# kuailehaha/liuzhou

Measured on AMD Instinct MI355X. Metric: self-play positions/sec (fixed sims/move), higher is better.
Workload: dtype f16

## Files before the change

### liuzhou_amd/csrc/lz_engine.hip

```cpp
#include <hip/hip_runtime.h>
#include <hip/amd_detail/amd_hip_unsafe_atomics.h>
#include <math.h>
#include <stdint.h>

#include <mutex>

#include "lz_rng.h"
#include "lz_tree_dev.h"

namespace {

__global__ __launch_bounds__(kBlock) void pack_states_kernel(LzStateSoA s, int64_t B, Packed* __restrict__ out) {
    const int64_t i = (int64_t)blockIdx.x * kBlock + threadIdx.x;
    if (i >= B) return;
    State st;
    st.black = cells_equal(s.board + i * 36, 1);
    st.white = cells_equal(s.board + i * 36, -1);
    st.mb = cells_nonzero(s.marks_black + i * 36);
    st.mw = cells_nonzero(s.marks_white + i * 36);
    st.phase = (int)s.phase[i]; st.player = (int)s.current_player[i];
    st.pm_req = (int)s.pending_marks_required[i]; st.pm_rem = (int)s.pending_marks_remaining[i];
    st.pc_req = (int)s.pending_captures_required[i]; st.pc_rem = (int)s.pending_captures_remaining[i];
    st.forced = (int)s.forced_removals_done[i]; st.move_count = (int)s.move_count[i];
    st.msc = (int)s.moves_since_capture[i];
    out[i] = pack(st);
}

__global__ __launch_bounds__(kBlock) void packed_planes_kernel(const Packed* __restrict__ states, int64_t B,
                                                               float* __restrict__ out) {
    const int lane = lane_id();
    const int64_t g = (int64_t)blockIdx.x * kWavesPerBlock + __builtin_amdgcn_readfirstlane((int)(threadIdx.x >> 6));
    if (g >= B) return;
    const State s = unpack(states[g]);
    const bool blk = s.player == 1;
    const uint64_t own = blk ? s.black : s.white, opp = blk ? s.white : s.black;
    const uint64_t sm = blk ? s.mb : s.mw, om = blk ? s.mw : s.mb;
    float4* orow = reinterpret_cast<float4*>(out + g * 396);
    for (int j = lane; j < 99; j += kWave) {
        const int plane = j / 9, cell0 = (j - plane * 9) * 4;
        uint32_t bits;
        if (plane < 4) {
            const uint64_t src = plane == 0 ? own : plane == 1 ? opp : plane == 2 ? sm : om;
            bits = (uint32_t)(src >> cell0) & 0xFu;
        } else bits = (s.phase == plane - 3) ? 0xFu : 0u;
        orow[j] = make_float4((bits & 1) ? 1.f : 0.f, (bits & 2) ? 1.f : 0.f, (bits & 4) ? 1.f : 0.f, (bits & 8) ? 1.f : 0.f);
    }
}

__global__ __launch_bounds__(kBlock) void tree_begin_kernel(Tree t) {
    const int g = blockIdx.x * kBlock + threadIdx.x;
    if (g >= t.B) return;
    begin_game(t, g);
}


__global__ __launch_bounds__(kBlock) void pos_clear_kernel(int* __restrict__ tab, int64_t n) {
    for (int64_t i = (int64_t)blockIdx.x * kBlock + threadIdx.x; i < n / 4; i += (int64_t)gridDim.x * kBlock)
        reinterpret_cast<int4*>(tab)[i] = make_int4(-1, -1, -1, -1);
}

__global__ __launch_bounds__(kBlock) void tree_select_kernel(Tree t) {
    const int g = wave_game();
    if (g >= t.B) return;
    tree_select(t, g, lane_id(), load_root_info(t, g));
}


template <bool IS_ROOT, bool COMPACT = false>
__global__ __launch_bounds__(kBlock) void tree_expand_kernel(Tree t, const float* __restrict__ lp1,
                                                             const float* __restrict__ lp2,
                                                             const float* __restrict__ lpm,
                                                             const float* __restrict__ priors220,
                                                             const float* __restrict__ values,
                                                             const float* __restrict__ noise, int noise_stride,
                                                             float epsilon, int step) {
    LZ_EXPAND_SCRATCH(sc);
    const int g = wave_game();
    if (g >= t.B) return;
    ptrdiff_t o = 0;
    if (COMPACT) o = (ptrdiff_t)(t.leaf_kind[g] == kLeafExpand ? t.live_row[g] : 0) - g;
    tree_expand<IS_ROOT>(t, g, lane_id(), lp1 ? lp1 + o * 36 : nullptr, lp2 ? lp2 + o * 36 : nullptr,
                         lpm ? lpm + o * 36 : nullptr, priors220 ? priors220 + o * 220 : nullptr, values + o, noise,
                         noise_stride, epsilon, sc, nullptr, step);
}

constexpr int kScanBlock = 1024;
constexpr int kScanUnroll = 8;
__global__ __launch_bounds__(kScanBlock) void tree_live_scan_kernel(Tree t, unsigned long long* __restrict__ count) {
    __shared__ int wave_total[kScanBlock / kWave];
    const int tid = threadIdx.x, lane = tid & (kWave - 1), w = tid / kWave;
    const int rounds = (t.B + kScanBlock - 1) / kScanBlock;
    int cnt = 0;
    for (int r0 = 0; r0 < rounds; r0 += kScanUnroll) {
        int kind[kScanUnroll];
#pragma unroll
        for (int u = 0; u < kScanUnroll; ++u) {
            const int g = (r0 + u) * kScanBlock + tid;
            kind[u] = (r0 + u < rounds && g < t.B) ? t.leaf_kind[g] : kLeafInactive;
        }
#pragma unroll
        for (int u = 0; u < kScanUnroll; ++u) cnt += kind[u] == kLeafExpand ? 1 : 0;
    }
    int incl = cnt;
#pragma unroll
    for (int d = 1; d < kWave; d <<= 1) {
        const int v = __shfl_up(incl, d, kWave);
        if (lane >= d) incl += v;
    }
    if (lane == kWave - 1) wave_total[w] = incl;
    __syncthreads();
    int before = 0, total = 0;
    for (int i = 0; i < kScanBlock / kWave; ++i) { if (i < w) before += wave_total[i]; total += wave_total[i]; }
    int row = before + incl - cnt;
    for (int r0 = 0; r0 < rounds; r0 += kScanUnroll) {
        int kind[kScanUnroll];
        Packed st[kScanUnroll];
#pragma unroll
        for (int u = 0; u < kScanUnroll; ++u) {
            const int g = (r0 + u) * kScanBlock + tid;
            const bool in = r0 + u < rounds && g < t.B;
            kind[u] = in ? t.leaf_kind[g] : kLeafInactive;
            if (in) st[u] = load_state(&t.leaf_state[g]);
        }
#pragma unroll
        for (int u = 0; u < kScanUnroll; ++u) {
            if (kind[u] != kLeafExpand) continue;
            const int g = (r0 + u) * kScanBlock + tid;
            t.live_row[g] = row;
            t.live_state[row] = st[u];
            ++row;
        }
    }
    if (tid == 0) *count = (unsigned long long)total;
}

template <bool IS_ROOT, bool COMPACT = false>
__global__ __launch_bounds__(kBlock) void tree_expand_select_kernel(Tree t, const float* __restrict__ lp1,
                                                                    const float* __restrict__ lp2,
                                                                    const float* __restrict__ lpm,
                                                                    const float* __restrict__ values,
                                                                    const float* __restrict__ noise, int noise_stride,
                                                                    float epsilon, int step) {
#ifndef LZ_EXP_NO_TREE_PRIO
    __builtin_amdgcn_s_setprio(3);
#endif
    LZ_EXPAND_SCRATCH(sc);
    const int g = wave_game();
    if (g >= t.B) return;
    const int lane = lane_id();
    RootInfo root;
    ptrdiff_t o = 0;
    if (COMPACT) o = (ptrdiff_t)(t.leaf_kind[g] == kLeafExpand ? t.live_row[g] : 0) - g;
#ifdef LZ_EXP_TREE_STAMPS
    const unsigned long long lz_t0 = __builtin_readcyclecounter();
#endif
    tree_expand<IS_ROOT>(t, g, lane, lp1 + o * 36, lp2 + o * 36, lpm + o * 36, nullptr, values + o, noise, noise_stride,
                         epsilon, sc, &root, step, nullptr, nullptr LZ_TSTAMP_PASS);
    __threadfence_block();
    if (IS_ROOT) root = load_root_info(t, g);
    LZ_TSTAMP(g, 7)
    tree_select(t, g, lane, root, -1, -1, nullptr LZ_TSTAMP_PASS);
#ifdef LZ_EXP_TREE_STAMPS
    LZ_TADD(g, 19, 1)
#endif
}

constexpr int kSplitMaxGames = 8192;
template <bool COMPACT>
__global__ __launch_bounds__(kBlock) void tree_expand_select_split_kernel(Tree t, const float* __restrict__ lp1,
                                                                          const float* __restrict__ lp2,
                                                                          const float* __restrict__ lpm,
                                                                          const float* __restrict__ values, int step) {
    __builtin_amdgcn_s_setprio(3);
    LZ_EXPAND_SCRATCH(sc);
    __shared__ int s_flag[kWavesPerBlock / 2];
    const int wv = __builtin_amdgcn_readfirstlane((int)(threadIdx.x >> 6));
    const int pair = wv >> 1, role = wv & 1;
    const int g = blockIdx.x * (kWavesPerBlock / 2) + pair;
    const int lane = lane_id();
    if (role == 0 && lane == 0) s_flag[pair] = 0;
    __syncthreads();
    if (g >= t.B) return;
    volatile int* flag = &s_flag[pair];
    ptrdiff_t o = 0;
    if (COMPACT) o = (ptrdiff_t)(t.leaf_kind[g] == kLeafExpand ? t.live_row[g] : 0) - g;
    if (role == 0) {
        tree_expand<false, 1>(t, g, lane, lp1 + o * 36, lp2 + o * 36, lpm + o * 36, nullptr, values + o, nullptr, 0, 0.f, sc,
                              nullptr, step, flag);
        __builtin_amdgcn_fence(__ATOMIC_RELEASE, "workgroup");
        if (lane == 0) *flag = kSplitExpanded;
    } else {
        RootInfo root;
        SplitInfo split;
        tree_expand<false, 2>(t, g, lane, lp1 + o * 36, lp2 + o * 36, lpm + o * 36, nullptr, values + o, nullptr, 0, 0.f, sc,
                              &root, step, flag, &split);
        __threadfence_block();
        split_wait(flag, kSplitInputsRead);
        tree_select(t, g, lane, root, split.wait_edge, split.nolegal_edge, flag);
    }
}

constexpr int kWaveDepth = 160;
struct WaveArrays {
    int K, cap;
    int* path; int* path_len; int* leaf_kind; Packed* leaf_state; float* leaf_value; int* leaf_edge; int* leaf_parent;
    int* sims_done; int* unfinished;
    int* eval_row; Packed* eval_state; unsigned long long* eval_count;
    unsigned long long* eval_total;
    int max_back;
};
struct Level { int e0, ne_pl, parent_n, node; double last_sc; int last_k, in_edge; };
static_assert(sizeof(Level) == 32, "level record is 32 bytes");

__device__ __forceinline__ Tree slot_view(const Tree& t, const WaveArrays& w, int j) {
    Tree v = t;
    const size_t o = (size_t)j * t.B;
    v.path = w.path + o * w.cap; v.path_cap = w.cap; v.path_len = w.path_len + o; v.leaf_kind = w.leaf_kind + o;
    v.leaf_state = w.leaf_state + o; v.leaf_value = w.leaf_value + o; v.leaf_edge = w.leaf_edge + o;
    v.leaf_parent = w.leaf_parent + o;
    return v;
}

__device__ __forceinline__ void tree_select_wave(const Tree& t, const WaveArrays& w, int g, int lane,
                                                 const RootInfo& root, int sims, Level* stack, int* leaf_node,
                                                 int* leaf_act) {
    const int done = w.sims_done[g];
    int to_collect = sims - done;
    to_collect = to_collect < w.K ? to_collect : w.K;
    const bool live = t.root_terminal[g] == 0 && root.ne > 0 && to_collect > 0;
    const Node* nodes = t.nodes + (size_t)g * t.node_cap;
    const Edge* edges = t.edges;
    int found = 0;
    if (live) {
        int d = 0;
        int e0 = root.e0, ne = root.ne, parent_n = root.visits, node_player = root.player, node = 0;
        double last_sc = INFINITY;
        int last_k = -1;
        Edge mine[2];
        double sc[2] = {0.0, 0.0};
        bool loaded = false;
        int ups = 0;
        bool last_leaf = false;
        while (found < to_collect) {
            if (!loaded) {
                const double sq = sqrt((double)(parent_n > 1 ? parent_n : 1));
#pragma unroll
                for (int r = 0; r < 2; ++r) {
                    const int k = r * kWave + lane;
                    sc[r] = __builtin_nan("");
                    if (k < ne) {
                        mine[r] = load_edge(&edges[(size_t)(e0 + k)]);
                        const int n = edge_n(mine[r].n_info);
                        double q = 0.0;
                        if (n > 0) {
                            const double mv = mine[r].W / (double)n;
                            const int child_player = (edge_info(mine[r].n_info) & kInfoWhite) ? -1 : 1;
                            q = child_player == node_player ? mv : -mv;
                        }
                        const double u = t.c_puct * (double)mine[r].P * sq / (1.0 + (double)n);
                        sc[r] = q + u;
                    }
                }
                loaded = true;
            }
            double best = -INFINITY;
            int best_k = -1;
#pragma unroll
            for (int r = 0; r < 2; ++r) {
// ... 857 lines not shown
    if (d->num_games == 0) return LZ_OK;
    const Tree t = no_share(make_tree(d));
    if (is_root)
        hipLaunchKernelGGL(tree_expand_kernel<true>, dim3(gw(t.B)), dim3(kBlock), 0, as_stream(stream), t, lp1, lp2,
                           lpmc, priors220, values, noise, (int)noise_stride, epsilon, -1);
    else
        hipLaunchKernelGGL(tree_expand_kernel<false>, dim3(gw(t.B)), dim3(kBlock), 0, as_stream(stream), t, lp1, lp2,
                           lpmc, priors220, values, nullptr, 0, 0.f, -1);
    return st();
}

int lz_tree_finish(const LzTreeDesc* d, const float* temperatures, const float* target_temperatures,
                   float prior_pseudocount, const uint8_t* force_uniform, int sample_moves, const float* uniforms,
                   float* policy_dense,
                   int32_t* chosen_index, int32_t* chosen_code, uint8_t* chosen_valid, uint8_t* terminal_mask,
                   float* root_value, int32_t* child_count, int32_t* child_action, int32_t* child_visits,
                   float* child_prior, int64_t out_cap, void* stream) {
    if (!tree_ok(d) || !temperatures || !policy_dense || !chosen_index || !chosen_code || !chosen_valid ||
        !terminal_mask || !root_value || !child_count || !child_action || !child_visits || !child_prior || out_cap < 1)
        return LZ_ERR_ARG;
    if (d->num_games == 0) return LZ_OK;
    if (!(prior_pseudocount >= 0.f) || ((force_uniform || sample_moves) && !uniforms)) return LZ_ERR_ARG;
    hipLaunchKernelGGL(tree_finish_kernel, dim3(gw(d->num_games)), dim3(kBlock), 0, as_stream(stream), make_tree(d),
                       temperatures, target_temperatures, prior_pseudocount, force_uniform, sample_moves, uniforms, policy_dense, chosen_index, reinterpret_cast<int4*>(chosen_code),
                       chosen_valid, terminal_mask, root_value, child_count, child_action, child_visits, child_prior,
                       (int)out_cap);
    return st();
}

static long long* g_advance_ticks = nullptr;
int lz_debug_advance_ticks(int64_t* ticks) { g_advance_ticks = reinterpret_cast<long long*>(ticks); return LZ_OK; }

int lz_prof_aux_begin(int kind, void* stream);
int lz_prof_aux_end(int kind, void* stream, int64_t units);

int lz_tree_advance(const LzTreeDesc* d, const int32_t* played_action, const uint8_t* reset, int64_t next_sims,
                    int32_t* dropped, int32_t* pruned, void* stream) {
    if (!tree_ok(d) || next_sims < 0) return LZ_ERR_ARG;
    if (d->num_games == 0) return LZ_OK;
    const int words = (d->node_cap + kWave - 1) / kWave;
    if (words > kMarkWordsBig) return LZ_ERR_UNSUPPORTED;
    const int64_t rn = next_sims + 1;
    if (rn > d->node_cap) return LZ_ERR_ARG;
    if ((int64_t)d->chunk_cap * (d->edge_chunk - (kMaxChildren - 1)) < (int64_t)d->node_cap * kMaxChildren) return LZ_ERR_ARG;
    const bool big = words > kMarkWordsMax;
    const int wpb = big ? 1 : kWavesPerBlock;
    const size_t lds = (size_t)wpb * (words * (sizeof(uint64_t) + sizeof(int)) + 3 * kWave * sizeof(int));
    if (big) {
        static std::mutex mu;
        static bool configured[64] = {};
        int dev = 0;
        if (hipGetDevice(&dev) != hipSuccess || dev < 0 || dev >= 64) return LZ_ERR_LAUNCH;
        std::lock_guard<std::mutex> lk(mu);
        if (!configured[dev]) {
            const size_t most = (size_t)kMarkWordsBig * (sizeof(uint64_t) + sizeof(int)) + 3 * kWave * sizeof(int);
            if (hipFuncSetAttribute(reinterpret_cast<const void*>(tree_advance_kernel<1>),
                                    hipFuncAttributeMaxDynamicSharedMemorySize, (int)most) != hipSuccess) {
                (void)hipGetLastError();
                return LZ_ERR_LAUNCH;
            }
            configured[dev] = true;
        }
    }
    (void)lz_prof_aux_begin(1, stream);
    if (big)
        hipLaunchKernelGGL(tree_advance_kernel<1>, dim3((unsigned)d->num_games), dim3(kWave), lds, as_stream(stream), make_tree(d),
                           played_action, reset, (int)rn, words, dropped, pruned, g_advance_ticks);
    else
        hipLaunchKernelGGL(tree_advance_kernel<kWavesPerBlock>, dim3(gw(d->num_games)), dim3(kBlock), lds, as_stream(stream),
                           make_tree(d), played_action, reset, (int)rn, words, dropped, pruned, g_advance_ticks);
    (void)lz_prof_aux_end(1, stream, d->num_games);
    return st();
}

static int tree_search_impl(const LzTreeDesc* d, const LzNetDesc* net, int64_t sims, float* planes, float* lp1,
                            float* lp2, float* lpmc, float* values, const float* noise, int64_t noise_stride,
                            float epsilon, bool continue_trees, void* stream) {
    if (!tree_ok(d) || !net || sims < 0 || !lp1 || !lp2 || !lpmc || !values) return LZ_ERR_ARG;
    const int64_t B = d->num_games;
    if (B == 0) return LZ_OK;
    int rc = continue_trees ? LZ_OK : lz_tree_begin(d, stream);
    if (rc) return rc;
    (void)planes;
    const Tree t = split_step(B) ? no_share(make_tree(d)) : make_tree(d);
    if (t.live_count != nullptr) {
        if (d->live_count_cap < sims + 2) return LZ_ERR_ARG;
        hipLaunchKernelGGL(tree_live_scan_kernel, dim3(1), dim3(kScanBlock), 0, as_stream(stream), t, t.live_count);
        for (int64_t s = 0; s <= sims; ++s) {
            rc = lz_net_forward_packed_counted_f16(net, d->live_state, B, d->live_count + s, lp1, lp2, lpmc, nullptr, values,
                                                   stream);
            if (rc) return rc;
            if (s == sims) {
                if (s == 0)
                    hipLaunchKernelGGL((tree_expand_kernel<true, true>), dim3(gw(t.B)), dim3(kBlock), 0, as_stream(stream), t,
                                       lp1, lp2, lpmc, (const float*)nullptr, values, noise, (int)noise_stride, epsilon, (int)s);
                else
                    hipLaunchKernelGGL((tree_expand_kernel<false, true>), dim3(gw(t.B)), dim3(kBlock), 0, as_stream(stream), t,
                                       lp1, lp2, lpmc, (const float*)nullptr, values, (const float*)nullptr, 0, 0.f, (int)s);
            } else if (s == 0) {
                hipLaunchKernelGGL((tree_expand_select_kernel<true, true>), dim3(gw(t.B)), dim3(kBlock), 0, as_stream(stream),
                                   t, lp1, lp2, lpmc, values, noise, (int)noise_stride, epsilon, (int)s);
            } else {
                (void)lz_prof_aux_begin(0, stream);
                if (split_step(t.B))
                    hipLaunchKernelGGL((tree_expand_select_split_kernel<true>), dim3(gw2(t.B)), dim3(kBlock), 0,
                                       as_stream(stream), t, lp1, lp2, lpmc, values, (int)s);
                else
                    hipLaunchKernelGGL((tree_expand_select_kernel<false, true>), dim3(gw(t.B)), dim3(kBlock), 0, as_stream(stream),
                                       t, lp1, lp2, lpmc, values, nullptr, 0, 0.f, (int)s);
                (void)lz_prof_aux_end(0, stream, B);
            }
            if (s < sims)
                hipLaunchKernelGGL(tree_live_scan_kernel, dim3(1), dim3(kScanBlock), 0, as_stream(stream), t,
                                   t.live_count + (s + 1));
        }
        return st();
    }
    for (int64_t s = 0; s <= sims; ++s) {
        rc = lz_net_forward_packed_f16(net, d->leaf_state, B, lp1, lp2, lpmc, nullptr, values, stream);
        if (rc) return rc;
        if (s == sims) {
            if (s == 0)
                hipLaunchKernelGGL(tree_expand_kernel<true>, dim3(gw(t.B)), dim3(kBlock), 0, as_stream(stream), t, lp1, lp2,
                                   lpmc, (const float*)nullptr, values, noise, (int)noise_stride, epsilon, (int)s);
            else
                hipLaunchKernelGGL(tree_expand_kernel<false>, dim3(gw(t.B)), dim3(kBlock), 0, as_stream(stream), t, lp1, lp2,
                                   lpmc, (const float*)nullptr, values, (const float*)nullptr, 0, 0.f, (int)s);
        } else if (s == 0) {
            hipLaunchKernelGGL(tree_expand_select_kernel<true>, dim3(gw(t.B)), dim3(kBlock), 0, as_stream(stream), t, lp1,
                               lp2, lpmc, values, noise, (int)noise_stride, epsilon, (int)s);
        } else {
            (void)lz_prof_aux_begin(0, stream);
            if (split_step(t.B))
                hipLaunchKernelGGL((tree_expand_select_split_kernel<false>), dim3(gw2(t.B)), dim3(kBlock), 0, as_stream(stream),
                                   t, lp1, lp2, lpmc, values, (int)s);
            else
                hipLaunchKernelGGL(tree_expand_select_kernel<false>, dim3(gw(t.B)), dim3(kBlock), 0, as_stream(stream), t, lp1,
                                   lp2, lpmc, values, nullptr, 0, 0.f, (int)s);
            (void)lz_prof_aux_end(0, stream, B);
        }
    }
    return st();
}

#ifdef LZ_EXP_TREE_STAMPS
LZ_API int lz_exp_tree_stamps(unsigned long long* out32, int reset) {
    if (out32 && hipMemcpyFromSymbol(out32, HIP_SYMBOL(g_tree_stamps), 32 * sizeof(unsigned long long)) != hipSuccess) return LZ_ERR_LAUNCH;
    if (reset) {
        unsigned long long z[32] = {};
        if (hipMemcpyToSymbol(HIP_SYMBOL(g_tree_stamps), z, sizeof(z)) != hipSuccess) return LZ_ERR_LAUNCH;
    }
    return LZ_OK;
}
#endif

int64_t lz_tree_desc_bytes(void) { return (int64_t)sizeof(LzTreeDesc); }

int lz_root_prepare(const void* root_states, int64_t B, const float* lp1, const float* lp2, const float* lpmc,
                    const float* noise, float epsilon, int64_t* legal_index_mat, float* priors_mat,
                    int32_t* action_code_mat, uint8_t* valid_mask, int32_t* counts, uint8_t* terminal_mask,
                    float* leaf_mat, void* child_states, int32_t* child_ref, uint64_t* n_children,
                    int64_t child_capacity, int32_t* overflow, void* stream) {
    if (B < 0) return LZ_ERR_ARG;
    if (B == 0) return LZ_OK;
    if (!root_states || !lp1 || !lp2 || !lpmc || !legal_index_mat || !priors_mat || !action_code_mat || !valid_mask ||
        !counts || !terminal_mask || !leaf_mat || !child_states || !child_ref || !n_children || child_capacity < 0)
        return LZ_ERR_ARG;
    if (reinterpret_cast<uintptr_t>(action_code_mat) & 15) return LZ_ERR_ALIGN;
    hipLaunchKernelGGL(zero_u64_kernel, dim3(1), dim3(64), 0, as_stream(stream),
                       reinterpret_cast<unsigned long long*>(n_children));
    hipLaunchKernelGGL(root_prepare_kernel, dim3(gw(B)), dim3(kBlock), 0, as_stream(stream),
                       reinterpret_cast<const Packed*>(root_states), B, lp1, lp2, lpmc, noise, epsilon, legal_index_mat,
                       priors_mat, reinterpret_cast<int4*>(action_code_mat), valid_mask, counts, terminal_mask, leaf_mat,
                       reinterpret_cast<Packed*>(child_states), child_ref,
                       reinterpret_cast<unsigned long long*>(n_children), child_capacity, overflow);
    return st();
}

int lz_root_collect(const void* root_states, const void* child_states, const int32_t* child_ref,
                    const float* child_values, const uint64_t* n_children, int64_t capacity, float soft_value_k,
                    float* leaf_mat, void* stream) {
    if (capacity < 0) return LZ_ERR_ARG;
    if (capacity == 0) return LZ_OK;
    if (!root_states || !child_states || !child_ref || !child_values || !n_children || !leaf_mat) return LZ_ERR_ARG;
    hipLaunchKernelGGL(root_collect_kernel, dim3(1024), dim3(kBlock), 0, as_stream(stream),
                       reinterpret_cast<const Packed*>(root_states), reinterpret_cast<const Packed*>(child_states),
                       child_ref, child_values, reinterpret_cast<const unsigned long long*>(n_children), capacity,
                       soft_value_k, leaf_mat);
    return st();
}

int lz_root_topk_children(const void* root_states, int64_t B, const float* leaf_mat, const uint8_t* valid_mask,
                          const int32_t* action_code_mat, int64_t top_k, int32_t* top_slot, void* l2_states, void* stream) {
    if (B < 0 || top_k < 0 || top_k > kRootCap) return LZ_ERR_ARG;
    if (B == 0 || top_k == 0) return LZ_OK;
    if (!root_states || !leaf_mat || !valid_mask || !action_code_mat || !top_slot || !l2_states) return LZ_ERR_ARG;
    if (reinterpret_cast<uintptr_t>(action_code_mat) & 15) return LZ_ERR_ALIGN;
// ... 97 lines not shown
```

### liuzhou_amd/csrc/lz_tree_dev.h

```cpp
#pragma once
#include <hip/hip_runtime.h>
#include <hip/amd_detail/amd_hip_unsafe_atomics.h>
#include <math.h>
#include <stdint.h>

#include "lz_soa.h"
#include "lz_wave.h"

using namespace lz;

namespace {

constexpr int kWave = 64;
constexpr int kBlock = 256;
constexpr int kWavesPerBlock = 4;
constexpr int kMaxChildren = 72;

enum LeafKind : int { kLeafInactive = 0, kLeafExpand = 1, kLeafTerminal = 2, kLeafReusedRoot = 3, kLeafShared = 4 };
constexpr uint8_t kInfoWhite = 1;
constexpr uint8_t kInfoTerminal = 2;

struct Edge {
    double W;
    float P;
    uint32_t n_info;
    int32_t child;
    int32_t cbegin;
    uint8_t act;
    uint8_t cn;
    uint8_t pad[6];
};
static_assert(sizeof(Edge) == 32, "edge record is 32 bytes");
struct Node {
    Packed state;
    int32_t edge_begin, nedges;
    int32_t parent;
    int32_t old_begin;
};
static_assert(sizeof(Node) == 48, "node record is 48 bytes");
__device__ __forceinline__ int edge_n(uint32_t ni) { return (int)(ni & 0xFFFFFFu); }
__device__ __forceinline__ uint8_t edge_info(uint32_t ni) { return (uint8_t)(ni >> 24); }

struct Tree {
    int B, node_cap, chunk, path_cap, chunk_cap;
    const Packed* root_state;
    Node* nodes; Edge* edges;
    int* n_nodes; int* n_edges;
    int* chunk_list; int* n_chunks; int* free_chunks; int* pool_top;
    int* pool_stats;
    int* root_visits; double* root_W; float* root_init_value;
    int* path; int* path_len; int* leaf_kind; Packed* leaf_state; float* leaf_value;
    uint8_t* root_terminal; const uint8_t* active;
    int* leaf_edge; int* leaf_parent;
    double c_puct;
    int fast_select;
    int* trace_kind; Packed* trace_leaf; float* trace_heads; float* trace_priors; float* trace_value;
    int trace_cap;
    int* eval_count;
    Packed* live_state; int* live_row; unsigned long long* live_count;
    int* pos_index; float* node_value; int* leaf_src; int* share_count;
    int pos_slots, share;
};

typedef unsigned int u32x4 __attribute__((ext_vector_type(4)));
__device__ __forceinline__ Edge load_edge(const Edge* p) {
    const u32x4* q = reinterpret_cast<const u32x4*>(p);
    union U { u32x4 v[2]; Edge e; __device__ U() {} } u;
    u.v[0] = q[0]; u.v[1] = q[1];
    return u.e;
}
__device__ __forceinline__ Packed load_state(const Packed* p) {
    const u32x4* q = reinterpret_cast<const u32x4*>(p);
    union U { u32x4 v[2]; Packed s; __device__ U() {} } u;
    u.v[0] = q[0]; u.v[1] = q[1];
    return u.s;
}
constexpr uint32_t kPathFlip = 0x80000000u;

__device__ __forceinline__ int lane_id() { return threadIdx.x & 63; }
__device__ __forceinline__ int wave_game() {
    return blockIdx.x * kWavesPerBlock + __builtin_amdgcn_readfirstlane((int)(threadIdx.x >> 6));
}
__device__ __forceinline__ bool same_state(const Packed& a, const Packed& b) {
    return a.w0 == b.w0 && a.w1 == b.w1 && a.w2 == b.w2 && a.w3 == b.w3;
}
__device__ __forceinline__ uint32_t pos_hash(const Packed& s) {
    uint64_t h = s.w0 * 0x9E3779B97F4A7C15ull;
    h = (h ^ (h >> 29) ^ s.w1) * 0xBF58476D1CE4E5B9ull;
    h = (h ^ (h >> 31) ^ s.w2) * 0x94D049BB133111EBull;
    h = (h ^ (h >> 27) ^ s.w3) * 0x9E3779B97F4A7C15ull;
    return (uint32_t)(h >> 32);
}
struct PosWindow { int entry; int first_empty; uint32_t base; };
__device__ __forceinline__ PosWindow pos_window(const Tree& t, int g, const Packed& s, int nn, int lane) {
    const int* tab = t.pos_index + (size_t)g * t.pos_slots;
    const uint32_t mask = (uint32_t)t.pos_slots - 1u;
    PosWindow w;
    w.base = pos_hash(s) & mask;
    w.entry = tab[(w.base + (uint32_t)lane) & mask];
    const uint64_t em = __ballot(w.entry < 1 || w.entry >= nn);
    w.first_empty = em ? __ffsll((unsigned long long)em) - 1 : kWave;
    return w;
}
__device__ __forceinline__ int pos_find(const Tree& t, int g, const Packed& s, int nn, int lane) {
    const PosWindow w = pos_window(t, g, s, nn, lane);
    bool hit = false;
    if (lane < w.first_empty) hit = same_state(load_state(&t.nodes[(size_t)g * t.node_cap + w.entry].state), s);
    const uint64_t hm = __ballot(hit);
    return hm ? lzw::lane_bcast(w.entry, __ffsll((unsigned long long)hm) - 1) : -1;
}

#ifdef LZ_EXP_TREE_STAMPS
__device__ unsigned long long g_tree_stamps[32];
#define LZ_TSTAMP_ON(g) ((g) == 5)
#define LZ_TSTAMP(g, k) if (LZ_TSTAMP_ON(g)) { asm volatile("s_waitcnt vmcnt(0) lgkmcnt(0)" ::: "memory"); \
        if (lane_id() == 0) { atomicAdd(&g_tree_stamps[k], (unsigned long long)__builtin_readcyclecounter() - lz_t0); \
                              atomicAdd(&g_tree_stamps[20 + (k)], 1ull); } }
#define LZ_TSTAMP_ARG , unsigned long long lz_t0 = 0
#define LZ_TSTAMP_PASS , lz_t0
#define LZ_TCLOCK(g, var) unsigned long long var = 0; if (LZ_TSTAMP_ON(g)) { asm volatile("s_waitcnt vmcnt(0) lgkmcnt(0)" ::: "memory"); var = __builtin_readcyclecounter(); }
#define LZ_TADD(g, k, v) if (LZ_TSTAMP_ON(g) && lane_id() == 0) atomicAdd(&g_tree_stamps[k], (unsigned long long)(v));
#else
#define LZ_TSTAMP(g, k)
#define LZ_TCLOCK(g, var)
#define LZ_TADD(g, k, v)
#define LZ_TSTAMP_ARG
#define LZ_TSTAMP_PASS
#endif

__device__ __forceinline__ double terminal_value_for_mover(const State& s) {
    const int st = game_status(s);
    if (st == 1 || st == -1) return st == s.player ? 1.0 : -1.0;
    return 0.0;
}


__device__ __forceinline__ void release_chunks(const Tree& t, int g, int keep) {
    const int nc = t.n_chunks[g];
    if (nc > keep) {
        const int base = atomicAdd(t.pool_top, nc - keep);
        const int* list = t.chunk_list + (size_t)g * t.chunk_cap;
        for (int i = keep; i < nc; ++i) t.free_chunks[base + (i - keep)] = list[i];
    }
    t.n_chunks[g] = keep < nc ? keep : nc;
}
__device__ __forceinline__ void release_chunks_wave(const Tree& t, int g, int keep, int lane) {
    const int nc = t.n_chunks[g];
    if (nc > keep) {
        int base = 0;
        if (lane == 0) base = atomicAdd(t.pool_top, nc - keep);
        base = __builtin_amdgcn_readfirstlane(base);
        const int* list = t.chunk_list + (size_t)g * t.chunk_cap;
        for (int i = keep + lane; i < nc; i += kWave) t.free_chunks[base + (i - keep)] = list[i];
        if (lane == 0) t.n_chunks[g] = keep;
    }
}
__device__ __forceinline__ bool root_pending(const Tree& t, int g) {
    return t.n_nodes[g] == 1 && t.nodes[(size_t)g * t.node_cap].nedges < 0 && t.root_terminal[g] == 0;
}

__device__ __forceinline__ int take_chunk(const Tree& t, int g, bool for_root = false) {
    const int nc = t.n_chunks[g];
    if (nc >= t.chunk_cap) { atomicAdd(t.pool_stats, 1); return -1; }
    const int top = atomicSub(t.pool_top, 1) - 1;
    const int reserved = for_root ? 0 : __atomic_load_n(t.pool_stats + 2, __ATOMIC_RELAXED);
    if (top < reserved) { atomicAdd(t.pool_top, 1); atomicAdd(t.pool_stats, 1); return -1; }
    if (for_root && root_pending(t, g)) atomicSub(t.pool_stats + 2, 1);
    atomicMin(t.pool_stats + 1, top);
    const int cid = t.free_chunks[top];
    t.chunk_list[(size_t)g * t.chunk_cap + nc] = cid;
    t.n_chunks[g] = nc + 1;
    return cid * t.chunk;
}

__device__ __forceinline__ void begin_game(const Tree& t, int g, bool release = true) {
    const bool was_pending = root_pending(t, g);
    if (release) release_chunks(t, g, 0);
    const Packed rs = t.root_state[g];
    Node& root = t.nodes[(size_t)g * t.node_cap];
    root.state = rs;
    root.edge_begin = 0;
    root.nedges = -1;
    root.parent = -1;
    t.n_nodes[g] = 1;
    t.n_edges[g] = 0;
    t.root_visits[g] = 0;
    t.root_W[g] = 0.0;
    t.root_init_value[g] = 0.f;
// ... 74 lines not shown
                    }
                    const float s = q + cf * mine[r].P * sqf / (1.0f + (float)n);
                    fs[r] = s == s ? s : -INFINITY;
                }
            }
            const float b = fs[1] > fs[0] ? fs[1] : fs[0];
            const float m1 = lzw::wave_max_nonan(b);
            const uint64_t w0 = __ballot(fs[0] == m1), w1 = __ballot(fs[1] == m1);
            if (m1 > -INFINITY && m1 < INFINITY && __popcll(w0) + __popcll(w1) == 1 && __ballot(off_scale) == 0ull) {
                const int c = w0 ? __ffsll((unsigned long long)w0) - 1 : kWave + __ffsll((unsigned long long)w1) - 1;
                const float b2 = (c & 63) == lane ? (c < kWave ? fs[1] : fs[0]) : b;
                const float m2 = lzw::wave_max_nonan(b2);
                if (m1 - m2 > 1e-4f * (1.0f + fabsf(m1))) chosen = c;
            }
        }
        if (chosen < 0) {
            const double sq = sqrt((double)(parent_n > 1 ? parent_n : 1));
            double best = -INFINITY;
            int best_k = -1;
#pragma unroll
            for (int r = 0; r < 2; ++r) {
                if (r == 1 && ne <= kWave) break;
                const int k = r * kWave + lane;
                if (k < ne) {
                    const int n = edge_n(mine[r].n_info);
                    double q = 0.0;
                    if (n > 0) {
                        const double mv = mine[r].W / (double)n;
                        const int child_player = (edge_info(mine[r].n_info) & kInfoWhite) ? -1 : 1;
                        q = child_player == node_player ? mv : -mv;
                    }
                    const double u = t.c_puct * (double)mine[r].P * sq / (1.0 + (double)n);
                    const double sc = q + u;
                    if (sc > best) { best = sc; best_k = k; }
                }
            }
            const double mx = lzw::wave_max(best);
            const uint64_t lo = __ballot(best_k >= 0 && best_k < kWave && best == mx);
            if (lo) chosen = __ffsll((unsigned long long)lo) - 1;
            else {
                const uint64_t hi = __ballot(best_k >= kWave && best == mx);
                if (!hi) break;
                chosen = kWave + __ffsll((unsigned long long)hi) - 1;
            }
        }
        chosen = __builtin_amdgcn_readfirstlane(chosen);
        const int src = chosen & 63;
        const bool up = chosen >= kWave;
        const uint32_t c_ni = (uint32_t)lzw::lane_bcast((int)(up ? mine[1].n_info : mine[0].n_info), src);
        int c_child = lzw::lane_bcast(up ? mine[1].child : mine[0].child, src);
        int c_begin = lzw::lane_bcast(up ? mine[1].cbegin : mine[0].cbegin, src);
        int c_meta = lzw::lane_bcast((int)(up ? mine[1].act : mine[0].act) | ((int)(up ? mine[1].cn : mine[0].cn) << 8), src);
        uint8_t info = edge_info(c_ni);
        if (e0 + chosen == wait_edge) {
            split_wait(flag, kSplitExpanded);
            const Edge fresh = load_edge(&run[chosen]);
            c_child = fresh.child; c_begin = fresh.cbegin;
            c_meta = (int)fresh.act | ((int)fresh.cn << 8);
        }
        if (e0 + chosen == nolegal_edge) info |= kInfoTerminal;
        const int child_player = (info & kInfoWhite) ? -1 : 1;
#ifdef LZ_EXP_TREE_STAMPS
        { LZ_TCLOCK(g, lv_t2) LZ_TADD(g, 17, lv_t2 - lv_t0) LZ_TADD(g, 18, 1) }
#endif
        leaf_edge = e0 + chosen;
        if (lane == 0) path[depth] = leaf_edge | (child_player != node_player ? (int)kPathFlip : 0);
        ++depth;
        if (info & kInfoTerminal) {
            kind = kLeafTerminal;
            term_value = (float)((int)((info >> 2) & 3) - 1);
            break;
        }
        if (c_child < 0) { kind = kLeafExpand; leaf_action = c_meta & 0xFF; break; }
        node_state = load_state(&nodes[c_child].state);
        parent_n = edge_n(c_ni);
        node_player = child_player;
        node = c_child;
        e0 = c_begin;
        ne = c_meta >> 8;
        if (depth >= t.path_cap - 1) break;
    }
    LZ_TSTAMP(g, 8)
    Packed leaf_packed{};
    int src = -1;
    if (kind == kLeafExpand) {
        State leaf = unpack(node_state);
        int kd, p, q2, ex;
        index_to_code(leaf.phase, leaf_action, kd, p, q2, ex);
        apply_legal(leaf, kd, p, q2);
        leaf_packed = pack(leaf);
        if (t.share) {
            src = pos_find(t, g, leaf_packed, t.n_nodes[g], lane);
            if (src > 0) kind = kLeafShared;
        }
    }
    if (lane == 0) {
        t.path_len[g] = depth;
        t.leaf_kind[g] = kind;
        t.leaf_value[g] = term_value;
        t.leaf_edge[g] = leaf_edge;
        t.leaf_parent[g] = node;
        if (kind == kLeafExpand || kind == kLeafShared) t.leaf_state[g] = leaf_packed;
        if (kind == kLeafShared) t.leaf_src[g] = src;
    }
    LZ_TSTAMP(g, 9)
}

struct ExpandScratch { float* val; int* act; };
constexpr int kExpandScratchBytes = 80 * 8;
#define LZ_EXPAND_SCRATCH(name)                                                            \
    __shared__ float name##_val[kWavesPerBlock][80];                                      \
    __shared__ int name##_act[kWavesPerBlock][80];                                        \
    const int name##_wv = __builtin_amdgcn_readfirstlane((int)(threadIdx.x >> 6));        \
    const ExpandScratch name = {name##_val[name##_wv], name##_act[name##_wv]}

struct SplitInfo { int wait_edge, nolegal_edge; };
template <bool IS_ROOT, int ROLE = 0>
__device__ __forceinline__ void tree_expand(const Tree& t, int g, int lane, const float* __restrict__ lp1,
                                            const float* __restrict__ lp2, const float* __restrict__ lpm,
                                            const float* __restrict__ priors220, const float* __restrict__ values,
                                            const float* __restrict__ noise, int noise_stride, float epsilon,
                                            ExpandScratch sc, RootInfo* root_after = nullptr, int step = -1,
                                            volatile int* flag = nullptr, SplitInfo* split = nullptr LZ_TSTAMP_ARG) {
    static_assert(ROLE == 0 || !IS_ROOT, "the root step is never split");
    LZ_TSTAMP(g, 0)
    const int kind = t.leaf_kind[g];
    Node* nodes = t.nodes + (size_t)g * t.node_cap;
    Edge* edges = t.edges;
    const int* path = t.path + (size_t)g * t.path_cap;
    RootInfo root{};
    int plen_ld = 0, leaf_edge = -1, leaf_parent = 0, nn_ld = 0, ne_ld = 0, path_entry = 0;
    double root_w = 0.0;
    float leaf_value_ld = 0.f, value_ld = 0.f;
    Packed leaf_packed = t.leaf_state[g];
    if (!IS_ROOT) {
        root = load_root_info(t, g);
        plen_ld = t.path_len[g];
        leaf_edge = t.leaf_edge[g];
        leaf_parent = t.leaf_parent[g];
        path_entry = lane < t.path_cap ? path[lane] : 0;
        root_w = t.root_W[g];
        leaf_value_ld = t.leaf_value[g];
    }
    nn_ld = t.n_nodes[g];
    ne_ld = t.n_edges[g];
    const bool shared = !IS_ROOT && ROLE == 0 && kind == kLeafShared;
    value_ld = shared ? 0.f : values[g];
    const bool indexed = !IS_ROOT && ROLE != 2 && t.pos_index != nullptr;
    PosWindow pw{0, kWave, 0u};
    if (indexed) pw = pos_window(t, g, leaf_packed, nn_ld, lane);
    int src_begin = 0;
    if (shared) {
        const int src = t.leaf_src[g];
        value_ld = t.node_value[(size_t)g * t.node_cap + src];
        src_begin = nodes[src].edge_begin;
    }
    if (root_after != nullptr) *root_after = root;
    if (ROLE == 1) {
        asm volatile("s_waitcnt vmcnt(0)" ::: "memory");
        if (lane == 0) *flag = kSplitInputsRead;
    }
    if (ROLE == 2) { split->wait_edge = -1; split->nolegal_edge = -1; }
    LZ_TSTAMP(g, 1)
    const bool tracing = ROLE != 2 && t.trace_kind != nullptr && step >= 0 && step < t.trace_cap;
    const size_t tslot = tracing ? (size_t)step * (size_t)t.B + (size_t)g : 0;
    if (tracing) {
        if (lane == 0) { t.trace_kind[tslot] = kind; t.trace_leaf[tslot] = leaf_packed; t.trace_value[tslot] = value_ld; }
        for (int a = lane; a < 220; a += kWave) t.trace_priors[tslot * 220 + a] = 0.f;
    }
    if (kind == kLeafInactive) return;
    if (kind == kLeafReusedRoot) {
        if (IS_ROOT && noise != nullptr) {
            const int ne = nodes[0].nedges, e0 = nodes[0].edge_begin;
            if (ne > 1) {
                const float keep = (float)(1.0 - (double)epsilon);
                float pr[2]; bool ok[2];
#pragma unroll
                for (int r = 0; r < 2; ++r) {
                    const int k = r * kWave + lane;
                    ok[r] = k < ne;
                    pr[r] = ok[r] ? keep * edges[(size_t)(e0 + k)].P + epsilon * noise[(size_t)g * noise_stride + k] : 0.f;
                }
                float psum = 0.f;
#pragma unroll
                for (int r = 0; r < 2; ++r) {
                    uint64_t m = __ballot(ok[r]);
                    while (m) {
                        const int l = __builtin_amdgcn_readfirstlane(__ffsll((unsigned long long)m) - 1);
                        psum += lzw::lane_bcast(pr[r], l);
                        m &= m - 1;
                    }
                }
                const float denom = psum < 1e-8f ? 1e-8f : psum;
#pragma unroll
                for (int r = 0; r < 2; ++r)
                    if (ok[r]) edges[(size_t)(e0 + r * kWave + lane)].P = pr[r] / denom;
            }
        }
        return;
    }
    const int plen = IS_ROOT ? 0 : plen_ld;
    double backup_value = 0.0;

    if (kind == kLeafTerminal) {
        backup_value = (double)leaf_value_ld;
    } else {
        if (shared) { if (t.share_count != nullptr && lane == 0) t.share_count[g] += 1; }
        else if (ROLE != 2 && t.eval_count != nullptr && lane == 0) t.eval_count[g] += 1;
        const State s = unpack(leaf_packed);
        const Legal L = legal_actions(s, 0);
        const int n = legal_count(L);
        if (ROLE == 2) {
            backup_value = n == 0 ? -1.0 : (double)value_ld;
            if (n == 0) split->nolegal_edge = leaf_edge; else split->wait_edge = leaf_edge;
        } else if (n == 0) {
            backup_value = -1.0;
            if (lane == 0) {
                if (IS_ROOT) {
                    if (root_pending(t, g)) atomicSub(t.pool_stats + 2, 1);
                    nodes[0].nedges = 0; t.root_terminal[g] = 1; t.root_init_value[g] = -1.f;
                }
                else atomicOr(&edges[(size_t)leaf_edge].n_info, (uint32_t)kInfoTerminal << 24);
            }
        } else {
            float h1 = 0.f, h2 = 0.f, hm = 0.f;
            const bool heads = priors220 == nullptr;
            if (heads && lane < kCells && !shared) {
                h1 = lp1[(size_t)g * 36 + lane]; h2 = lp2[(size_t)g * 36 + lane]; hm = lpm[(size_t)g * 36 + lane];
                if (tracing) {
                    float* th = t.trace_heads + tslot * 108;
                    th[lane] = h1; th[36 + lane] = h2; th[72 + lane] = hm;
                }
            }
            float val[4]; int slot[4]; bool lg[4];
            int base = 0;
            float mx = -INFINITY;
// ... 3 lines not shown
                lg[it] = a < 217 && legal_bit(L, a);
                val[it] = 0.f; slot[it] = 0;
                const uint64_t bal = __ballot(lg[it]);
                if (bal == 0) continue;
                slot[it] = base + __popcll(bal & ((1ull << lane) - 1ull));
                base += __popcll(bal);
                int from = 0, dest = 0, cell = 0;
                if (a >= 36 && a < 180) { from = (a - 36) >> 2; dest = move_dest(from, (a - 36) & 3); dest = dest < 0 ? 0 : (dest > 35 ? 35 : dest); }
                else if (a >= 180 && a < 216) cell = a - 180;
                else if (a < 36) cell = a;
                float x;
                if (heads) {
                    const float p1d = __shfl(h1, dest), p2f = __shfl(h2, from), p1c = __shfl(h1, cell), pmc = __shfl(hm, cell);
                    x = a < 36 ? p1c : a < 180 ? (p2f + p1d) : a < 216 ? pmc : 0.f;
                } else {
                    x = lg[it] ? priors220[(size_t)g * 220 + a] : 0.f;
                }
                val[it] = x;
                if (heads && lg[it]) mx = fmaxf(mx, x);
            }
            if (heads) {
                mx = lzw::wave_max(mx);
                float sum = 0.f;
#pragma unroll
                for (int it = 0; it < 4; ++it) { val[it] = lg[it] ? expf(val[it] - mx) : 0.f; sum += val[it]; }
                sum = lzw::wave_sum(sum);
#pragma unroll
                for (int it = 0; it < 4; ++it) val[it] = val[it] / sum;
            }
            if (tracing) {
#pragma unroll
                for (int it = 0; it < 4; ++it)
                    if (lg[it]) t.trace_priors[tslot * 220 + it * kWave + lane] = val[it];
            }
            if (IS_ROOT && noise != nullptr && n > 1) {
                const float keep = (float)(1.0 - (double)epsilon);
#pragma unroll
                for (int it = 0; it < 4; ++it)
                    if (lg[it]) val[it] = keep * val[it] + epsilon * noise[(size_t)g * noise_stride + slot[it]];
            }
            LZ_TSTAMP(g, 2)
#pragma unroll
            for (int it = 0; it < 4; ++it)
                if (lg[it]) { sc.val[slot[it]] = val[it]; sc.act[slot[it]] = it * kWave + lane; }
            __builtin_amdgcn_fence(__ATOMIC_RELEASE, "wavefront");
            __builtin_amdgcn_wave_barrier();
            __builtin_amdgcn_fence(__ATOMIC_ACQUIRE, "wavefront");
            float cval[2]; int cact[2];
#pragma unroll
            for (int r = 0; r < 2; ++r) {
                const int k = r * kWave + lane;
                cval[r] = k < n ? sc.val[k] : 0.f;
                cact[r] = k < n ? sc.act[k] : 0;
            }
            float psum = 0.f;
            if (shared) {
#pragma unroll
                for (int r = 0; r < 2; ++r) {
                    const int k = r * kWave + lane;
                    cval[r] = k < n ? edges[(size_t)(src_begin + k)].P : 0.f;
                }
                psum = 1.f;
            } else {
#pragma unroll 4
                for (int k = 0; k < n; ++k) psum += lzw::lane_bcast(k < kWave ? cval[0] : cval[1], k & 63);
            }
            const bool bad = !(psum > 0.f) || !isfinite(psum);
            LZ_TSTAMP(g, 3)
            int node_id = 0, e0 = 0;
            if (lane == 0) {
                e0 = ne_ld;
                const int off = e0 & (t.chunk - 1);
                if (off == 0 || off + n > t.chunk) e0 = take_chunk(t, g, IS_ROOT);
                if (e0 >= 0) {
                    t.n_edges[g] = e0 + n;
                    if (IS_ROOT) node_id = 0;
                    else {
                        node_id = nn_ld; t.n_nodes[g] = node_id + 1;
                        Edge& in = edges[(size_t)leaf_edge];
                        in.child = node_id; in.cbegin = e0; in.cn = (uint8_t)n;
                        nodes[node_id].state = leaf_packed;
                        nodes[node_id].parent = leaf_parent;
                        if (t.node_value != nullptr) t.node_value[(size_t)g * t.node_cap + node_id] = value_ld;
                        if (indexed && !shared && pw.first_empty < kWave)
                            t.pos_index[(size_t)g * t.pos_slots + ((pw.base + (uint32_t)pw.first_empty) & ((uint32_t)t.pos_slots - 1u))] = node_id;
                    }
                    nodes[node_id].edge_begin = e0;
                    nodes[node_id].nedges = n;
                }
                if (IS_ROOT) t.root_init_value[g] = value_ld;
            }
            e0 = __builtin_amdgcn_readfirstlane(e0);
            node_id = __builtin_amdgcn_readfirstlane(node_id);
            const int n_write = e0 >= 0 ? n : 0;
            LZ_TSTAMP(g, 4)
            Edge* new_run = edges + (size_t)(e0 >= 0 ? e0 : 0);
            for (int r = 0; r < (n_write > kWave ? 2 : 1); ++r) {
                const int k = r * kWave + lane;
                if (k >= n_write) continue;
                const int a = r == 0 ? cact[0] : cact[1];
                State c = s;
                int kd, p, q2, ex;
                index_to_code(s.phase, a, kd, p, q2, ex);
                apply_legal(c, kd, p, q2);
                uint8_t info = c.player < 0 ? kInfoWhite : 0;
                if (game_status(c) != 0) {
                    const int tv = (int)terminal_value_for_mover(c);
                    info |= kInfoTerminal | (uint8_t)((tv + 1) << 2);
                }
                Edge rec;
                rec.W = 0.0;
                rec.P = shared ? (r == 0 ? cval[0] : cval[1]) : bad ? (1.0f / (float)n) : ((r == 0 ? cval[0] : cval[1]) / psum);
                rec.n_info = (uint32_t)info << 24;
                rec.child = -1;
                rec.cbegin = 0;
                rec.act = (uint8_t)a;
                rec.cn = 0;
                rec.pad[0] = rec.pad[1] = rec.pad[2] = rec.pad[3] = rec.pad[4] = rec.pad[5] = 0;
                new_run[k] = rec;
            }
            backup_value = (double)value_ld;
            LZ_TSTAMP(g, 5)
        }
    }
    if (IS_ROOT || ROLE == 1) return;
    if (plen > 0) {
        int flips_above = 0;
        for (int hi = plen; hi > 0; hi -= kWave) {
            const int lo = hi > kWave ? hi - kWave : 0;
            const int j = lo + lane;
            const bool in = j < hi;
            const uint32_t pe = !in ? 0u : (lo == 0 ? (uint32_t)path_entry : (uint32_t)path[j]);
            const uint64_t F = __ballot(in && (pe & kPathFlip) != 0u);
            const int above = in ? __popcll(F >> (lane + 1)) : 0;
            if (in) {
                Edge* e = &edges[(size_t)(pe & ~kPathFlip)];
                const double v = ((above + flips_above) & 1) ? -backup_value : backup_value;
                atomicAdd(&e->n_info, 1u);
                unsafeAtomicAdd(&e->W, v);
            }
            flips_above += __popcll(F);
        }
        root.visits += 1;
        if (lane == 0) {
            t.root_visits[g] = root.visits;
            t.root_W[g] = root_w + ((flips_above & 1) ? -backup_value : backup_value);
        }
        if (root_after != nullptr) root_after->visits = root.visits;
    }
    LZ_TSTAMP(g, 6)
}

inline hipStream_t as_stream(void* s) { return reinterpret_cast<hipStream_t>(s); }
inline int st() { return hipGetLastError() == hipSuccess ? LZ_OK : LZ_ERR_LAUNCH; }

Tree make_tree(const LzTreeDesc* d) {
    Tree t;
    t.B = (int)d->num_games; t.node_cap = d->node_cap; t.chunk = d->edge_chunk; t.path_cap = d->path_cap;
    t.chunk_cap = d->chunk_cap;
    t.chunk_list = d->chunk_list; t.n_chunks = d->n_chunks; t.free_chunks = d->free_chunks; t.pool_top = d->pool_top;
    t.pool_stats = d->pool_stats;
    t.root_state = reinterpret_cast<const Packed*>(d->root_state);
    t.nodes = reinterpret_cast<Node*>(d->nodes);
    t.edges = reinterpret_cast<Edge*>(d->edges);
    t.n_nodes = d->n_nodes; t.n_edges = d->n_edges; t.root_visits = d->root_visits; t.root_W = d->root_w;
    t.root_init_value = d->root_init_value;
    t.path = d->path; t.path_len = d->path_len; t.leaf_kind = d->leaf_kind;
    t.leaf_state = reinterpret_cast<Packed*>(d->leaf_state); t.leaf_value = d->leaf_value;
    t.root_terminal = d->root_terminal; t.active = d->active;
    t.leaf_edge = d->leaf_edge; t.leaf_parent = d->leaf_parent;
    t.c_puct = d->exploration_weight;
    { const char* e = getenv("LZ_TREE_F32SEL"); t.fast_select = (e && e[0] == '1'); }
    const bool tr = d->trace_cap > 0 && d->trace_kind && d->trace_leaf && d->trace_heads && d->trace_priors && d->trace_value;
    t.trace_kind = tr ? d->trace_kind : nullptr;
    t.trace_leaf = tr ? reinterpret_cast<Packed*>(d->trace_leaf) : nullptr;
    t.trace_heads = tr ? d->trace_heads : nullptr;
    t.trace_priors = tr ? d->trace_priors : nullptr;
    t.trace_value = tr ? d->trace_value : nullptr;
    t.trace_cap = tr ? (int)d->trace_cap : 0;
    t.eval_count = d->eval_count;
    const bool live = d->live_state && d->live_row && d->live_count && d->live_count_cap > 0;
    t.live_state = live ? reinterpret_cast<Packed*>(d->live_state) : nullptr;
    t.live_row = live ? d->live_row : nullptr;
    t.live_count = live ? reinterpret_cast<unsigned long long*>(d->live_count) : nullptr;
    const bool pos = d->pos_index && d->node_value && d->leaf_src && d->pos_slots >= kWave &&
                     (d->pos_slots & (d->pos_slots - 1)) == 0;
    t.pos_index = pos ? d->pos_index : nullptr;
    t.node_value = pos ? d->node_value : nullptr;
    t.leaf_src = pos ? d->leaf_src : nullptr;
    t.pos_slots = pos ? (int)d->pos_slots : 0;
    t.share_count = d->share_count;
    { const char* e = getenv("LZ_TREE_SHARE"); t.share = pos && !tr && !(e && e[0] == '0') ? 1 : 0; }
    return t;
}
inline Tree no_share(Tree t) { t.share = 0; return t; }
bool tree_ok(const LzTreeDesc* d) {
    return d && d->num_games >= 0 && d->node_cap >= 2 && d->path_cap >= 3 &&
           d->edge_chunk >= 128 && (d->edge_chunk & (d->edge_chunk - 1)) == 0 && d->chunk_cap >= 1 &&
           d->pool_chunks >= 1 && (d->pool_chunks + 1) * (int64_t)d->edge_chunk <= (int64_t)1 << 31 &&
           d->pool_chunks >= d->num_games &&
           d->chunk_list && d->n_chunks && d->free_chunks && d->pool_top && d->pool_stats &&
           d->root_state && d->nodes && d->edges && d->n_nodes && d->n_edges &&
           d->root_visits && d->root_w && d->root_init_value && d->path && d->path_len && d->leaf_kind &&
           d->leaf_state && d->leaf_value && d->root_terminal && d->leaf_edge && d->leaf_parent;
}

}
```

Measured before the change: 11400.

## Parallelize live-leaf compaction across blocks and reuse select-time position-index slot

```diff
diff --git a/liuzhou_amd/csrc/lz_engine.hip b/liuzhou_amd/csrc/lz_engine.hip
--- a/liuzhou_amd/csrc/lz_engine.hip
+++ b/liuzhou_amd/csrc/lz_engine.hip
@@ -78,7 +78,7 @@
     const int g = wave_game();
     if (g >= t.B) return;
     ptrdiff_t o = 0;
-    if (COMPACT) o = (ptrdiff_t)(t.leaf_kind[g] == kLeafExpand ? t.live_row[g] : 0) - g;
+    if (COMPACT) o = (ptrdiff_t)t.live_row[g] - g;
     tree_expand<IS_ROOT>(t, g, lane_id(), lp1 ? lp1 + o * 36 : nullptr, lp2 ? lp2 + o * 36 : nullptr,
                          lpm ? lpm + o * 36 : nullptr, priors220 ? priors220 + o * 220 : nullptr, values + o, noise,
                          noise_stride, epsilon, sc, nullptr, step);
@@ -124,14 +124,81 @@
         }
 #pragma unroll
         for (int u = 0; u < kScanUnroll; ++u) {
+            const int g = (r0 + u) * kScanBlock + tid;
+            if (r0 + u < rounds && g < t.B) t.live_row[g] = kind[u] == kLeafExpand ? row : 0;
             if (kind[u] != kLeafExpand) continue;
-            const int g = (r0 + u) * kScanBlock + tid;
-            t.live_row[g] = row;
             t.live_state[row] = st[u];
             ++row;
         }
     }
     if (tid == 0) *count = (unsigned long long)total;
+}
+
+constexpr int kListBlock = 1024;
+constexpr int kListWaves = kListBlock / kWave;
+constexpr int kListMaxRounds = 256;
+inline bool list_build_ok(const Tree& t) {
+    return (t.B + kScanBlock - 1) / kScanBlock <= kListMaxRounds && (reinterpret_cast<uintptr_t>(t.leaf_kind) & 15) == 0;
+}
+inline unsigned list_groups(int B) { return (unsigned)(((B < kScanBlock ? B : kScanBlock) + kWave - 1) / kWave); }
+__global__ __launch_bounds__(kListBlock) void tree_live_list_kernel(Tree t, unsigned long long* __restrict__ count) {
+    __shared__ uint64_t col_mask[kListMaxRounds];
+    __shared__ int wave_before[kListWaves];
+    const int tid = threadIdx.x, lane = tid & (kWave - 1);
+    const int wv = __builtin_amdgcn_readfirstlane(tid >> 6);
+    const int rounds = (t.B + kScanBlock - 1) / kScanBlock;
+    const int c0 = blockIdx.x * kWave;
+    const int q = c0 >> 2, groups = rounds * q;
+    int before = 0;
+    for (int i0 = tid; i0 < groups; i0 += 4 * kListBlock) {
+        int4 k[4];
+#pragma unroll
+        for (int u = 0; u < 4; ++u) {
+            const int i = i0 + u * kListBlock;
+            const int r = i / (q > 0 ? q : 1);
+            const int g = r * kScanBlock + 4 * (i - r * q);
+            k[u] = make_int4(kLeafInactive, kLeafInactive, kLeafInactive, kLeafInactive);
+            if (i < groups) {
+                if (g + 3 < t.B) k[u] = *reinterpret_cast<const int4*>(t.leaf_kind + g);
+                else {
+                    if (g < t.B) k[u].x = t.leaf_kind[g];
+                    if (g + 1 < t.B) k[u].y = t.leaf_kind[g + 1];
+                    if (g + 2 < t.B) k[u].z = t.leaf_kind[g + 2];
+                }
+            }
+        }
+#pragma unroll
+        for (int u = 0; u < 4; ++u)
+            before += (k[u].x == kLeafExpand) + (k[u].y == kLeafExpand) + (k[u].z == kLeafExpand) + (k[u].w == kLeafExpand);
+    }
+    const int g_first = wv * kScanBlock + c0 + lane;
+    Packed st_first{};
+    if (wv < rounds && g_first < t.B) st_first = load_state(&t.leaf_state[g_first]);
+    for (int r = wv; r < rounds; r += kListWaves) {
+        const int g = r * kScanBlock + c0 + lane;
+        const uint64_t m = __ballot(g < t.B && t.leaf_kind[g] == kLeafExpand);
+        if (lane == 0) col_mask[r] = m;
+    }
+    before = lzw::wave_incl_scan(before);
+    if (lane == kWave - 1) wave_before[wv] = before;
+    __syncthreads();
+    int base = 0;
+    for (int i = 0; i < kListWaves; ++i) base += wave_before[i];
+    const uint64_t below = (1ull << lane) - 1ull;
+    int col_row = base;
+    for (int r = 0; r < rounds; ++r) col_row += __popcll(col_mask[r] & below);
+    for (int r = 0; r < rounds; ++r) {
+        const bool live = (col_mask[r] >> lane) & 1ull;
+        if (r % kListWaves == wv) {
+            const int g = r * kScanBlock + c0 + lane;
+            if (g < t.B) {
+                t.live_row[g] = live ? col_row : 0;
+                if (live) t.live_state[col_row] = r == wv ? st_first : load_state(&t.leaf_state[g]);
+            }
+        }
+        col_row += live ? 1 : 0;
+    }
+    if (blockIdx.x == gridDim.x - 1 && wv == 0 && lane == kWave - 1) *count = (unsigned long long)col_row;
 }
 
 template <bool IS_ROOT, bool COMPACT = false>
@@ -150,7 +217,7 @@
     const int lane = lane_id();
     RootInfo root;
     ptrdiff_t o = 0;
-    if (COMPACT) o = (ptrdiff_t)(t.leaf_kind[g] == kLeafExpand ? t.live_row[g] : 0) - g;
+    if (COMPACT) o = (ptrdiff_t)t.live_row[g] - g;
 #ifdef LZ_EXP_TREE_STAMPS
     const unsigned long long lz_t0 = __builtin_readcyclecounter();
 #endif
@@ -183,7 +250,7 @@
     if (g >= t.B) return;
     volatile int* flag = &s_flag[pair];
     ptrdiff_t o = 0;
-    if (COMPACT) o = (ptrdiff_t)(t.leaf_kind[g] == kLeafExpand ? t.live_row[g] : 0) - g;
+    if (COMPACT) o = (ptrdiff_t)t.live_row[g] - g;
     if (role == 0) {
         tree_expand<false, 1>(t, g, lane, lp1 + o * 36, lp2 + o * 36, lpm + o * 36, nullptr, values + o, nullptr, 0, 0.f, sc,
                               nullptr, step, flag);
@@ -1207,10 +1274,21 @@
     int rc = continue_trees ? LZ_OK : lz_tree_begin(d, stream);
     if (rc) return rc;
     (void)planes;
-    const Tree t = split_step(B) ? no_share(make_tree(d)) : make_tree(d);
+    const char* ref_env = getenv("LZ_TREE_LIST_REF");
+    const bool ref = ref_env && ref_env[0] == '1';
+    Tree t = split_step(B) ? no_share(make_tree(d)) : make_tree(d);
+    t.sel_slot = t.share && !ref ? 1 : 0;
     if (t.live_count != nullptr) {
         if (d->live_count_cap < sims + 2) return LZ_ERR_ARG;
-        hipLaunchKernelGGL(tree_live_scan_kernel, dim3(1), dim3(kScanBlock), 0, as_stream(stream), t, t.live_count);
+        const bool list = !ref && list_build_ok(t);
+        auto build_list = [&](unsigned long long* count) {
+            if (list)
+                hipLaunchKernelGGL(tree_live_list_kernel, dim3(list_groups(t.B)), dim3(kListBlock), 0, as_stream(stream), t,
+                                   count);
+            else
+                hipLaunchKernelGGL(tree_live_scan_kernel, dim3(1), dim3(kScanBlock), 0, as_stream(stream), t, count);
+        };
+        build_list(t.live_count);
         for (int64_t s = 0; s <= sims; ++s) {
             rc = lz_net_forward_packed_counted_f16(net, d->live_state, B, d->live_count + s, lp1, lp2, lpmc, nullptr, values,
                                                    stream);
@@ -1235,9 +1313,7 @@
                                        t, lp1, lp2, lpmc, values, nullptr, 0, 0.f, (int)s);
                 (void)lz_prof_aux_end(0, stream, B);
             }
-            if (s < sims)
-                hipLaunchKernelGGL(tree_live_scan_kernel, dim3(1), dim3(kScanBlock), 0, as_stream(stream), t,
-                                   t.live_count + (s + 1));
+            if (s < sims) build_list(t.live_count + (s + 1));
         }
         return st();
     }
diff --git a/liuzhou_amd/csrc/lz_tree_dev.h b/liuzhou_amd/csrc/lz_tree_dev.h
--- a/liuzhou_amd/csrc/lz_tree_dev.h
+++ b/liuzhou_amd/csrc/lz_tree_dev.h
@@ -60,6 +60,7 @@
     Packed* live_state; int* live_row; unsigned long long* live_count;
     int* pos_index; float* node_value; int* leaf_src; int* share_count;
     int pos_slots, share;
+    int sel_slot;
 };
 
 typedef unsigned int u32x4 __attribute__((ext_vector_type(4)));
@@ -102,8 +103,12 @@
     w.first_empty = em ? __ffsll((unsigned long long)em) - 1 : kWave;
     return w;
 }
-__device__ __forceinline__ int pos_find(const Tree& t, int g, const Packed& s, int nn, int lane) {
+__device__ __forceinline__ int pos_slot(const Tree& t, const PosWindow& w) {
+    return w.first_empty < kWave ? (int)((w.base + (uint32_t)w.first_empty) & ((uint32_t)t.pos_slots - 1u)) : -1;
+}
+__device__ __forceinline__ int pos_find(const Tree& t, int g, const Packed& s, int nn, int lane, int* slot) {
     const PosWindow w = pos_window(t, g, s, nn, lane);
+    *slot = pos_slot(t, w);
     bool hit = false;
     if (lane < w.first_empty) hit = same_state(load_state(&t.nodes[(size_t)g * t.node_cap + w.entry].state), s);
     const uint64_t hm = __ballot(hit);
@@ -344,7 +349,7 @@
     }
     LZ_TSTAMP(g, 8)
     Packed leaf_packed{};
-    int src = -1;
+    int src = -1, slot = -1;
     if (kind == kLeafExpand) {
         State leaf = unpack(node_state);
         int kd, p, q2, ex;
@@ -352,7 +357,7 @@
         apply_legal(leaf, kd, p, q2);
         leaf_packed = pack(leaf);
         if (t.share) {
-            src = pos_find(t, g, leaf_packed, t.n_nodes[g], lane);
+            src = pos_find(t, g, leaf_packed, t.n_nodes[g], lane, &slot);
             if (src > 0) kind = kLeafShared;
         }
     }
@@ -364,6 +369,7 @@
         t.leaf_parent[g] = node;
         if (kind == kLeafExpand || kind == kLeafShared) t.leaf_state[g] = leaf_packed;
         if (kind == kLeafShared) t.leaf_src[g] = src;
+        else if (kind == kLeafExpand && t.sel_slot) t.leaf_src[g] = slot;
     }
     LZ_TSTAMP(g, 9)
 }
@@ -407,13 +413,17 @@
     nn_ld = t.n_nodes[g];
     ne_ld = t.n_edges[g];
     const bool shared = !IS_ROOT && ROLE == 0 && kind == kLeafShared;
-    value_ld = shared ? 0.f : values[g];
+    const float value_any = values[g];
+    value_ld = shared ? 0.f : value_any;
     const bool indexed = !IS_ROOT && ROLE != 2 && t.pos_index != nullptr;
-    PosWindow pw{0, kWave, 0u};
-    if (indexed) pw = pos_window(t, g, leaf_packed, nn_ld, lane);
+    const bool hinted = indexed && t.sel_slot;
+    const int src_ld = hinted ? t.leaf_src[g] : 0;
+    int ins_slot = -1;
+    if (indexed && !hinted) ins_slot = pos_slot(t, pos_window(t, g, leaf_packed, nn_ld, lane));
+    if (hinted) ins_slot = src_ld;
     int src_begin = 0;
     if (shared) {
-        const int src = t.leaf_src[g];
+        const int src = hinted ? src_ld : t.leaf_src[g];
         value_ld = t.node_value[(size_t)g * t.node_cap + src];
         src_begin = nodes[src].edge_begin;
     }
@@ -583,8 +593,8 @@
                         nodes[node_id].state = leaf_packed;
                         nodes[node_id].parent = leaf_parent;
                         if (t.node_value != nullptr) t.node_value[(size_t)g * t.node_cap + node_id] = value_ld;
-                        if (indexed && !shared && pw.first_empty < kWave)
-                            t.pos_index[(size_t)g * t.pos_slots + ((pw.base + (uint32_t)pw.first_empty) & ((uint32_t)t.pos_slots - 1u))] = node_id;
+                        if (indexed && !shared && ins_slot >= 0)
+                            t.pos_index[(size_t)g * t.pos_slots + ins_slot] = node_id;
                     }
                     nodes[node_id].edge_begin = e0;
                     nodes[node_id].nedges = n;
@@ -692,9 +702,10 @@
     t.pos_slots = pos ? (int)d->pos_slots : 0;
     t.share_count = d->share_count;
     { const char* e = getenv("LZ_TREE_SHARE"); t.share = pos && !tr && !(e && e[0] == '0') ? 1 : 0; }
+    t.sel_slot = 0;
     return t;
 }
-inline Tree no_share(Tree t) { t.share = 0; return t; }
+inline Tree no_share(Tree t) { t.share = 0; t.sel_slot = 0; return t; }
 bool tree_ok(const LzTreeDesc* d) {
     return d && d->num_games >= 0 && d->node_cap >= 2 && d->path_cap >= 3 &&
            d->edge_chunk >= 128 && (d->edge_chunk & (d->edge_chunk - 1)) == 0 && d->chunk_cap >= 1 &&
```

Measured after the change: 11560, median of 6. 1.4% higher.
